# maxdoblas/QuickEd

Hardware: AMD Instinct MI355X
Metric: alignments/sec + GCUPS, 10kb x 10kb 5%-error pairs (higher is better)
Workload: dtype u64; 1 GPU; banded_score, DEVICE-RESIDENT inputs: 100000 pairs/GPU x 10000 bp @ 0.05 error, bandwidth 15 %, seeded generator (SURVEY 8d), ASCII already in HBM when the clock starts, results left in HBM (end-to-end rates: e2e); pairs_per_gpu=100000, length=10000, bandwidth=15, parallelism=pairs sharded over 1 GPU(s), no data-path collective

## Files before the change

### quicked_amd/csrc/qe_kernels.hip

```cpp
#include <type_traits>
#include <hip/hip_runtime.h>
#include "qe_types.h"
#include "qe_bounded.h"
#include "qe_search.h"
#include "qe_tags.h"
#include "qe_check.h"

namespace qe {

#define QE_ONES (~(u64)0)
#define QE_WAVE_IN_BLOCK() ((int)(threadIdx.x >> 6))
#define QE_GROUP_INDEX() ((int)(blockIdx.x * (blockDim.x >> 6) + (threadIdx.x >> 6)))
extern __shared__ uint4 qe_dyn_lds[];

__device__ __forceinline__ u32 lo32(u64 x) { return (u32)x; }
__device__ __forceinline__ u32 hi32(u64 x) { return (u32)(x >> 32); }
__device__ __forceinline__ u64 mk64(u32 lo, u32 hi) { return ((u64)hi << 32) | lo; }

__device__ __forceinline__ int64_t tile_elem(int col, int slot, int nslots) {
    return ((int64_t)(col >> 3) * nslots + slot) * 512 + (col & 7);
}

__device__ __forceinline__ int wave_min(int v) {
#pragma unroll
// ... 250 lines not shown
                u32 inP, inM;
                if (k == 0) { inP = __builtin_amdgcn_ubfe(hp, c, 1); inM = __builtin_amdgcn_ubfe(hm, c, 1); }
                else {
                    inP = (gP[k - 1] & 1u) | top[k];
                    inM = (gM[k - 1] & 1u) & ~top[k];
                }
                u32 phhi, mhhi;
                block_step_core(elo, ehi, Plo[k], Phi[k], Mlo[k], Mhi[k], inP, inM, phhi, mhhi);
                gP[k] = __builtin_amdgcn_alignbit(gP[k], phhi, 31);
                gM[k] = __builtin_amdgcn_alignbit(gM[k], mhhi, 31);
                if (k + 1 == K) asm("" : "+v"(Plo[k]) : "v"(gP[k]), "v"(gM[k]));
                if ((c & 15) == 15) {
                    if (act[k]) {
                        uint4* q = st + (int64_t)(2 * half + (c >> 4) + 1) * st_stride + k * 64;
                        if (c == 31 && half == 1) q = (k == 0) ? stl_first : stl + k * 64;
                        *q = make_uint4(Plo[k], Phi[k], Mlo[k], Mhi[k]);
                    }
                }
            }
        }
#pragma unroll
        for (int k = 0; k < K; ++k) {
            const u32 rP = __builtin_bitreverse32(gP[k]), rM = __builtin_bitreverse32(gM[k]);
            if (half) { oPhi[k] = rP; oMhi[k] = rM; } else { oPlo[k] = rP; oMlo[k] = rM; }
        }
    }
#pragma unroll
    for (int k = 0; k < K; ++k) {
        P[k] = mk64(Plo[k], Phi[k]); M[k] = mk64(Mlo[k], Mhi[k]);
        oP[k] = mk64(oPlo[k], oPhi[k]); oM[k] = mk64(oMlo[k], oMhi[k]);
    }
}

template <int K>
__device__ __forceinline__ void slots_pass(int nl, int i, int r, u64* Pv, u64* Mv, const int32_t* Srd, int32_t* Swr, int64_t stride,
                                           const u64* pp, int p0, u64 T0, u64 T1, u64& hinP, u64& hinM, u32& adv) {
    u64 P[K], M[K], a[K], b[K];
    int sc[K], v0[K];
#pragma unroll
    for (int k = 0; k < K; ++k) {
        P[k] = 0; M[k] = 0; a[k] = 0; b[k] = 0; sc[k] = 0;
        if (k < nl) {
            u64 nn;
            P[k] = Pv[(int64_t)(i + k) * stride]; M[k] = Mv[(int64_t)(i + k) * stride]; sc[k] = Srd[(int64_t)(r + k) * stride];
            load_planes(pp, p0 + 64 * (r + k), a[k], b[k], nn);
        }
        v0[k] = __popcll(P[k]) - __popcll(M[k]);
    }
    u64 houtP, houtM;
    run64_skew<K>(P, M, a, b, T0, T1, hinP, hinM, houtP, houtM);
    if (nl > 0) {
        int d = __popcll(houtP) - __popcll(houtM);
#pragma unroll
        for (int k = K - 1; k >= 0; --k) {
            if (k < nl) {
                Swr[(int64_t)(r + k) * stride] = sc[k] + d;
                Pv[(int64_t)(i + k - 1) * stride] = P[k]; Mv[(int64_t)(i + k - 1) * stride] = M[k];
            }
            d -= (__popcll(P[k]) - __popcll(M[k])) - v0[k];
        }
        adv += 64u * (u32)nl;
    }
    hinP = houtP; hinM = houtM;
}

__device__ __forceinline__ void run64_win2(u64& P0, u64& M0, u64& P1, u64& M1, u64 a0, u64 b0, u64 a1, u64 b1, u64 T0, u64 T1,
                                           u64 hinP, bool patch, u64 Eq_x, u64& gP, u64& gM, uint4* st, int st_stride) {
    const u32 a0lo = lo32(a0), a0hi = hi32(a0), b0lo = lo32(b0), b0hi = hi32(b0);
    const u32 a1lo = lo32(a1), a1hi = hi32(a1), b1lo = lo32(b1), b1hi = hi32(b1);
    u32 P0lo = lo32(P0), P0hi = hi32(P0), M0lo = lo32(M0), M0hi = hi32(M0);
    u32 P1lo = lo32(P1), P1hi = hi32(P1), M1lo = lo32(M1), M1hi = hi32(M1);
    u32 oPlo = 0, oPhi = 0, oMlo = 0, oMhi = 0;
#pragma unroll 1
    for (int half = 0; half < 2; ++half) {
        const u32 t0 = half ? hi32(T0) : lo32(T0), t1 = half ? hi32(T1) : lo32(T1);
        const u32 hp = half ? hi32(hinP) : lo32(hinP);
        u32 g0P = 0, g0M = 0;
        u32 m0[32], m1[32];
#pragma unroll
        for (int s = 0; s < 33; ++s) {
            if (s < 32) {
                m0[s] = (u32)__builtin_amdgcn_sbfe((int)t0, s, 1);
                m1[s] = (u32)__builtin_amdgcn_sbfe((int)t1, s, 1);
            }
            if (s >= 1) {
                const int c = s - 1;
                if ((c & 7) == 0) st[(4 * half + (c >> 3)) * st_stride] = make_uint4(P1lo, P1hi, M1lo, M1hi);
                u32 inP = g0P & 1u, inM = g0M & 1u;
                if (c == 31 && half == 1 && patch) {
// ... 343 lines not shown
    Geom g;
    const int kend = abs(n - m) + 1;
    g.cutoff = max(max(kend, cutoff_in), 65);
    g.diff = m - n;
    const int rel = (g.cutoff - abs(g.diff) + 1) / 2;
    if (g.diff >= 0) {
        g.prolog = (rel + 63) / 64;
        g.ebb = (rel + g.diff + 63) / 64 + 1 + g.prolog;
    } else {
        g.prolog = (rel - g.diff + 63) / 64;
        g.ebb = (rel + 63) / 64 + 1 + g.prolog;
    }
    g.fin = g.prolog * 64 + g.diff;
    return g;
}

struct GroupWs {
    u64* Pv; u64* Mv; int32_t* S; int16_t* cf; int16_t* cl;
};
__device__ __forceinline__ GroupWs group_ws(uint8_t* ws, int64_t off, int ns, int nrows, int nch) {
    GroupWs w;
    uint8_t* p = ws + off;
    w.Pv = (u64*)p;              p += (int64_t)(ns + 1) * 64 * 8;
    w.Mv = (u64*)p;              p += (int64_t)(ns + 1) * 64 * 8;
    w.S = (int32_t*)p;           p += (int64_t)nrows * 64 * 4;
    w.cf = (int16_t*)p;          p += (int64_t)nch * 64 * 2;
    w.cl = (int16_t*)p;
    return w;
}

#ifndef QE_FILL_K
#define QE_FILL_K 3
#endif
template <bool FILL>
__global__ __launch_bounds__(512) void k_banded(BandedArgs A) {
    const int g = QE_GROUP_INDEX(), lane = threadIdx.x & 63, t = g * 64 + lane;
    if (g * 64 >= A.T.ntasks) return;
    int pair = (t < A.T.ntasks) ? A.T.pair[t] : -1;
    if (A.only_if != nullptr && pair >= 0 && A.only_if[t] == 0) pair = -1;
    const bool valid = pair >= 0;
    if (!__any(valid)) return;
    int m = 1, n = 1, p0 = 0, t0 = 0, cut_in = 0, tfin = 0, prune = 0x7fffffff;
    const u64* pp = A.P.pl_p;
    const u64* tp = A.P.pl_t;
    u32 fl = 0;
    if (valid) {
        m = A.T.m[t]; n = A.T.n[t]; p0 = A.T.p0[t]; t0 = A.T.t0[t];
        cut_in = A.T.cutoff[t];
        tfin = FILL ? n : A.T.tfin[t];
        if (!FILL && A.prune != nullptr) prune = A.prune[t];
        pp = A.P.pl_p + A.P.pl_p_off[pair];
        tp = A.P.pl_t + A.P.pl_t_off[pair];
        fl = A.P.flags[pair];
    }
    const bool hasN = (fl & FLAG_HAS_N) != 0;
    const Geom G = band_geometry(m, n, cut_in);
    const int thr = prune < cut_in ? prune : G.cutoff;
    const int nw = (m + 63) >> 6;
    const bool fgeom = FILL || A.fill_geom != 0;
    const int nsl = fgeom ? G.ebb : ((G.cutoff + 63) >> 6) + 1;
    const int stop_row = fgeom ? nw - 1 : nw;
    const int lvl_last = (m - 1) & 63;
    int first = G.prolog, last = nsl - 1, pos_v = -G.prolog, pos_h = 0;
    int max_row_init = nsl - 1;
    u32 adv = 0;

    const int gns = A.g_nslots[g], gnr = A.g_nrows[g], gnch = A.g_nch[g];
    const GroupWs W = group_ws(A.ws, A.g_ws_off[g], gns, gnr, gnch);
    u64* const Pv = W.Pv + 64 + lane;
    u64* const Mv = W.Mv + 64 + lane;
    int32_t* const S = W.S + lane;
    uint4* const cp = FILL ? A.mat + A.g_mat_off[g] + lane : nullptr;
    const int64_t cps = (int64_t)gns * 64;
    uint4* const hw = FILL ? cp + (int64_t)QE_CPC * gnch * cps : nullptr;

    for (int s = 0; s < gns; ++s) {
        if (valid && s < nsl) {
            Pv[(int64_t)s * 64] = QE_ONES;
            Mv[(int64_t)s * 64] = 0;
            S[(int64_t)s * 64] = 64 * (s + 1);
            if (FILL) cp[(int64_t)s * 64] = make_uint4(~0u, ~0u, 0u, 0u);
        }
    }
    if (FILL && valid) { W.cf[lane] = (int16_t)first; W.cl[lane] = (int16_t)last; }

    const int nfull = tfin >> 6, tail = tfin & 63;
    const int my_chunks = valid ? nfull + (tail ? 1 : 0) : 0;
    const int wave_chunks = wave_max(my_chunks);

    for (int k = 0; k < wave_chunks; ++k) {
        const int ncols = (k < nfull) ? 64 : ((k == nfull) ? tail : 0);
        const bool on = valid && ncols > 0;
        u64 T0 = 0, T1 = 0, TN = 0;
        if (on) load_planes(tp, t0 + 64 * k, T0, T1, TN);
        const int rhi = min(last, nw - 1 - pos_v);
        const int fmin = wave_min(on ? first : 0x7fffffff), fmax = wave_max(on ? first : -0x7fffffff);
        const bool rel = A.lane_rel != 0 && fmin < fmax;
        const int ib = rel ? (on ? first : 0) : 0;
        const int i0 = rel ? 0 : fmin;
        const int i1 = rel ? wave_max(on ? rhi - first : -0x7fffffff) : wave_max(on ? rhi : -0x7fffffff);
        u64 hinP = QE_ONES, hinM = 0;
        u64 qP = 0, qM = 0, qa0 = 0, qb0 = 0, qa1 = 0, qb1 = 0;
        int qS = 0, qi = -0x7fffffff;
        const int psh = p0 & 63;
        const bool unaligned = __any(psh != 0);
        auto prefetch = [&](int j) {
            const int jc = min(max(j, 0), gns - 1), rc = min(max(j + pos_v, 0), gnr - 1), rp = min(max(j + pos_v, 0), nw);
            qP = Pv[(int64_t)jc * 64]; qM = Mv[(int64_t)jc * 64]; qS = S[(int64_t)rc * 64];
            const u64* w = pp + 3 * (int64_t)((p0 >> 6) + rp);
            qa0 = w[0]; qb0 = w[1];
            if (unaligned) { qa1 = w[3]; qb1 = w[4]; }
            qi = j;
        };
        if (FILL) prefetch(i0 + ib);
        for (int x = i0; x <= i1; ++x) {
            const int i = x + ib;
            const bool act = on && i >= first && i <= rhi;
            const int r = i + pos_v;
            if (!FILL) {
                const int lo = on ? first : 0x7fffffff, hi_ = on ? rhi : -0x7fffffff;
                const bool plain = !(on && (ncols != 64 || hasN));
                int nl = 0;
                auto planned = [&](int K) {
                    bool bad;
                    nl = pass_plan(i, K, lo, hi_, r, nw, plain, A.score_masked != 0, bad);
                    return !__any(bad);
                };
                if (i == first) { hinP = QE_ONES; hinM = 0; }
                if (x + 3 <= i1 && planned(4)) { slots_pass<4>(nl, i, r, Pv, Mv, S, S, 64, pp, p0, T0, T1, hinP, hinM, adv); x += 3; continue; }
                if (x + 1 <= i1 && planned(2)) { slots_pass<2>(nl, i, r, Pv, Mv, S, S, 64, pp, p0, T0, T1, hinP, hinM, adv); x += 1; continue; }
            }
            if (FILL && QE_FILL_K > 1 && A.fill_multi && x + QE_FILL_K - 1 <= i1) {
                constexpr int K = QE_FILL_K;
                bool actk[K], slowk = false;
                u32 topk[K];
#pragma unroll
                for (int q = 0; q < K; ++q) {
                    actk[q] = on && (i + q) >= first && (i + q) <= rhi;
                    topk[q] = ((i + q) == first) ? 1u : 0u;
                    slowk |= actk[q] && (ncols != 64 || hasN || (i + q + pos_v) == nw - 1);
                }
                if (!__any(slowk)) {
                    u64 P[K], M[K], a[K], b[K], oP[K], oM[K];
                    int sc[K];
#pragma unroll
                    for (int q = 0; q < K; ++q) {
                        P[q] = 0; M[q] = 0; a[q] = 0; b[q] = 0; sc[q] = 0;
                        if (actk[q]) {
                            u64 nn;
                            P[q] = Pv[(int64_t)(i + q) * 64]; M[q] = Mv[(int64_t)(i + q) * 64]; sc[q] = S[(int64_t)(r + q) * 64];
                            load_planes(pp, p0 + 64 * (r + q), a[q], b[q], nn);
                        }
                    }
                    if (i == first) { hinP = QE_ONES; hinM = 0; }
                    uint4* const st0 = cp + (int64_t)(QE_CPC * k) * cps + (int64_t)i * 64;
                    uint4* const stl0 = cp + (int64_t)(QE_CPC * k + QE_CPC) * cps + (int64_t)(i - 1) * 64;
                    run64_skew_fill<K>(P, M, a, b, T0, T1, hinP, hinM, oP, oM, actk, topk, st0, cps,
                                       (i == 0) ? st0 + QE_CPC * cps : stl0, stl0);
#pragma unroll
                    for (int q = 0; q < K; ++q) {
                        if (actk[q]) {
                            const u64 iP = (q == 0) ? hinP : (topk[q] ? QE_ONES : oP[q > 0 ? q - 1 : 0]);
                            const u64 iM = (q == 0) ? hinM : (topk[q] ? (u64)0 : oM[q > 0 ? q - 1 : 0]);
                            hw[((int64_t)k * gns + (i + q)) * 64] = make_uint4(lo32(iP), hi32(iP), lo32(iM), hi32(iM));
                            S[(int64_t)(r + q) * 64] = sc[q] + __popcll(oP[q]) - __popcll(oM[q]);
                            Pv[(int64_t)(i + q - 1) * 64] = P[q]; Mv[(int64_t)(i + q - 1) * 64] = M[q];
                            adv += 64u;
                        }
                    }
                    hinP = oP[K - 1]; hinM = oM[K - 1];
                    x += K - 1;
                    continue;
                }
            }
            u64 P = 0, M = 0, a = 0, b = 0, nn = 0;
            int sc = 0;
            if (FILL) {
                if (qi != i) prefetch(i);
                if (act) {
                    P = qP; M = qM; sc = qS;
                    a = (qa0 >> psh) | ((qa1 << 1) << (63 - psh));
                    b = (qb0 >> psh) | ((qb1 << 1) << (63 - psh));
                    if (hasN || r == nw - 1) load_planes(pp, p0 + 64 * r, a, b, nn);
                }
                prefetch(i + 1);
            } else if (act) {
                P = Pv[(int64_t)i * 64];
                M = Mv[(int64_t)i * 64];
                sc = S[(int64_t)r * 64];
                load_planes(pp, p0 + 64 * r, a, b, nn);
            }
            if (i == first) { hinP = QE_ONES; hinM = 0; }
            const bool lastblk = (r == nw - 1);
            uint4* st = nullptr; uint4* st_last = nullptr;
            if (FILL) {
                st = cp + (int64_t)(QE_CPC * k) * cps + (int64_t)i * 64;
                st_last = cp + (int64_t)(QE_CPC * k + QE_CPC) * cps + (int64_t)(i - 1) * 64;
                if (i == 0) st_last = st + QE_CPC * cps;
                if (act) hw[((int64_t)k * gns + i) * 64] = make_uint4(lo32(hinP), hi32(hinP), lo32(hinM), hi32(hinM));
            }
            u64 houtP, houtM, sP, sM;
            const bool slow = act && (ncols != 64 || hasN || lastblk);
            if (!__any(slow)) {
                run64_fast<FILL ? 2 : 0, true>(P, M, a, b, T0, T1, hinP, hinM, houtP, houtM, act, st, cps, st_last);
                sP = houtP; sM = houtM;
            } else {
                run64_general<FILL ? 2 : 0>(P, M, a, b, nn, T0, T1, TN, hinP, hinM, houtP, houtM, sP, sM,
                                            lastblk ? lvl_last : 63, act ? ncols : 0, true, st, cps, st_last);
            }
            if (act) {
                sc += __popcll(sP) - __popcll(sM);
                S[(int64_t)r * 64] = sc;
                const int64_t dst = (ncols == 64) ? (int64_t)(i - 1) * 64 : (int64_t)i * 64;
                Pv[dst] = P;
                Mv[dst] = M;
                adv += (u32)ncols;
            }
            hinP = houtP; hinM = houtM;
        }
        if (on && ncols == 64) {
            const bool c1 = (first + 2 < last) && (G.fin > 64 * (first + 1));
            bool cut_lo = false;
            if (c1) cut_lo = S[(int64_t)(first + pos_v + 1) * 64] + (G.fin - 64 * (first + 1)) > thr;
            if (cut_lo && pos_h >= G.prolog) first++;
            else if (!cut_lo && pos_h < G.prolog) first--;
            Pv[(int64_t)last * 64] = QE_ONES;
            Mv[(int64_t)last * 64] = 0;
            if (FILL) cp[(int64_t)(QE_CPC * k + QE_CPC) * cps + (int64_t)last * 64] = make_uint4(~0u, ~0u, 0u, 0u);
            const int pos = last + pos_v;
            S[(int64_t)(pos + 1) * 64] = S[(int64_t)pos * 64] + 64;
            max_row_init = max(max_row_init, pos + 1);
            const bool c2 = (first + 2 < last) && (64 * (last - 1) > G.fin);
            bool cut_hi = false;
            if (c2) cut_hi = S[(int64_t)(last + pos_v - 1) * 64] + (64 * (last - 1) - G.fin) > thr;
            if (cut_hi || (pos_v + last >= stop_row)) last--;
            pos_v++;
            pos_h++;
            if (FILL) { W.cf[(int64_t)pos_h * 64 + lane] = (int16_t)first; W.cl[(int64_t)pos_h * 64 + lane] = (int16_t)last; }
        }
    }
    if (valid) {
        const int row = nw - 1;
        int score = -1;
        if (row <= max_row_init) {
            score = S[(int64_t)row * 64];
            if (m & 63) score -= 64 - (m & 63);
        }
        A.o_score[t] = score;
        A.o_first[t] = first;
        A.o_last[t] = last;
        A.o_posv[t] = pos_v;
        A.o_maxrow[t] = max_row_init;
        A.o_adv[t] = adv;
    }
}

template __global__ void k_banded<false>(BandedArgs);
template __global__ void k_banded<true>(BandedArgs);

#define QE_HAVE_K_BOUNDED_DIAG 1
__global__ __launch_bounds__(256) void k_bounded_diag(BoundedArgs A) {
    const int g = QE_GROUP_INDEX(), lane = threadIdx.x & 63, t = g * 64 + lane;
    if (g * 64 >= A.T.ntasks) return;
    const int pair = (t < A.T.ntasks) ? A.T.pair[t] : -1;
    const bool valid = pair >= 0;
    if (!__any(valid)) return;
    int m = 1, n = 1, bound = 0;
    const u64* pp = A.P.pl_p;
    const u64* tp = A.P.pl_t;
    BoundedDiag S;
    S.Pv = S.Mv = S.wa = S.wb = S.wn = S.xa = S.xb = S.xn = S.force = S.track = 0; S.score = 0; S.dlo = 0;
    if (valid) {
        m = A.T.m[t]; n = A.T.n[t]; bound = A.T.cutoff[t];
        pp = A.P.pl_p + A.P.pl_p_off[pair];
        tp = A.P.pl_t + A.P.pl_t_off[pair];
        bounded_diag_init(S, pp, m, n, bound);
    }
    const int my_chunks = valid ? (n + 63) >> 6 : 0;
    const int wave_chunks = wave_max(my_chunks);
    u32 adv = 0;
    for (int k = 0; k < wave_chunks; ++k) {
        const int ncols = (k < my_chunks) ? min(64, n - 64 * k) : 0;
        const bool live = ncols > 0 && S.score <= bound;
        if (!__any(live)) break;
        if (live) {
            const u64* q = tp + 3 * (int64_t)k;
            const u64 T0 = q[0], T1 = q[1], TN = q[2];
            bounded_diag_chunk(S, pp, m, k, ncols, T0, T1, TN);
            adv += (u32)ncols;
        }
    }
// ... 3311 lines not shown
```

### quicked_amd/csrc/qe_pool.h

```cpp
#pragma once
#include <hip/hip_runtime.h>

#include <sys/syscall.h>
#include <unistd.h>

#include <algorithm>
#include <atomic>
#include <chrono>
#include <cstdio>
#include <cstdlib>
#include <cstring>
#include <memory>
#include <mutex>
#include <shared_mutex>
#include <thread>
#include <vector>

namespace qe {

struct HipError { hipError_t e; const char* what; int line; };
#define HIP_CHECK(expr)                                                             \
    do {                                                                            \
        hipError_t e__ = (expr);                                                    \
        if (e__ != hipSuccess) throw qe::HipError{e__, #expr, __LINE__};            \
    } while (0)

struct Chip {
    int cus = 256, simds = 1024;
    size_t slots2() const { return (size_t)simds * 2; }
    size_t frac2(double f) const { return (size_t)((double)simds * 2.0 * f); }
};
inline const Chip& chip(int device) {
    static Chip table[16];
    static std::once_flag once[16];
    const int d = (device >= 0 && device < 16) ? device : 0;
    std::call_once(once[d], [d] {
        int cus = 0;
        if (hipDeviceGetAttribute(&cus, hipDeviceAttributeMultiprocessorCount, d) == hipSuccess && cus > 0) { table[d].cus = cus; table[d].simds = cus * 4; }
        else (void)hipGetLastError();
    });
    return table[d];
}

enum class Sw : int {
    QuickedFast, QuickedEst, QuickedScorePass, FinishMerge, FinishMergePairs, Finishers, LaneRel, CoopG, CoopFillG, CoopLds,
    CoopTallFill, Wave, ScoreSys, Stage3Device, FormatWave, WindowedCp, WindowedQuad, WindowedSys, SplitBytes, FillSys, FillMulti,
    TraceSys, Trace, TracePool, OomWaitMs, BoundedDiag, ScoreNarrow, NarrowFit, NarrowPrune, ScoreMasked, TagsWave, SearchForm, SearchHitsWsKb, Count
};
struct SwitchDef { Sw sw; const char* name; long long dflt; };
inline constexpr SwitchDef switch_defs[] = {
    {Sw::QuickedFast, "QE_QUICKED_FAST", 1},           {Sw::QuickedEst, "QE_QUICKED_EST", 0},
    {Sw::QuickedScorePass, "QE_QUICKED_SCORE_PASS", -1},
    {Sw::FinishMerge, "QE_FINISH_MERGE", 4},           {Sw::FinishMergePairs, "QE_FINISH_MERGE_PAIRS", 8192},
    {Sw::Finishers, "QE_FINISHERS", 3},                {Sw::LaneRel, "QE_LANE_REL", 1},
    {Sw::CoopG, "QE_COOP_G", 1},                       {Sw::CoopFillG, "QE_COOP_FILL_G", 1},
    {Sw::CoopLds, "QE_COOP_LDS", 1},                   {Sw::CoopTallFill, "QE_COOP_TALL_FILL", 1},
    {Sw::Wave, "QE_WAVE", -1},                         {Sw::ScoreSys, "QE_SCORE_SYS", -1},
    {Sw::Stage3Device, "QE_STAGE3_DEVICE", -1},        {Sw::FormatWave, "QE_FORMAT_WAVE", -1},
    {Sw::WindowedCp, "QE_WINDOWED_CP", 1},             {Sw::WindowedQuad, "QE_WINDOWED_QUAD", -1},
    {Sw::WindowedSys, "QE_WINDOWED_SYS", -1},          {Sw::SplitBytes, "QE_SPLIT_BYTES", 1LL << 24},
    {Sw::FillSys, "QE_FILL_SYS", -1},                  {Sw::FillMulti, "QE_FILL_MULTI", 1},
    {Sw::TraceSys, "QE_TRACE_SYS", -1},                {Sw::Trace, "QE_TRACE", 0},
    {Sw::TracePool, "QE_TRACE_POOL", 0},               {Sw::OomWaitMs, "QE_OOM_WAIT_MS", 10000},
    {Sw::BoundedDiag, "QE_BOUNDED_DIAG", -1},
    {Sw::ScoreNarrow, "QE_SCORE_NARROW", -1},
    {Sw::NarrowFit, "QE_NARROW_FIT", -1},
    {Sw::NarrowPrune, "QE_NARROW_PRUNE", -1},
    {Sw::ScoreMasked, "QE_SCORE_MASKED", 1},
    {Sw::TagsWave, "QE_TAGS_WAVE", -1},
    {Sw::SearchForm, "QE_SEARCH_FORM", -1},
    {Sw::SearchHitsWsKb, "QE_SEARCH_HITS_WS_KB", 262144},
};
inline constexpr int switch_count = (int)Sw::Count;
constexpr bool switch_rows_in_order() {
    for (int i = 0; i < switch_count; ++i) if ((int)switch_defs[i].sw != i) return false;
    return true;
}
static_assert(sizeof(switch_defs) / sizeof(switch_defs[0]) == (size_t)switch_count && switch_rows_in_order(), "one row per switch, in the order of Sw");

struct SwitchTable {
    bool set[switch_count];
    long long value[switch_count];
    SwitchTable() {
        for (int i = 0; i < switch_count; ++i) {
            const char* e = getenv(switch_defs[i].name);
            set[i] = e != nullptr;
            value[i] = e ? strtoll(e, nullptr, 10) : switch_defs[i].dflt;
        }
    }
};
inline std::atomic<const SwitchTable*> g_switches{nullptr};
inline const SwitchTable& switches() {
    const SwitchTable* t = g_switches.load(std::memory_order_acquire);
    if (!t) {
        const SwitchTable* fresh = new SwitchTable();
        if (g_switches.compare_exchange_strong(t, fresh, std::memory_order_acq_rel)) t = fresh;
        else delete fresh;
    }
    return *t;
}
inline void switches_reload() { g_switches.store(new SwitchTable(), std::memory_order_release); }
// ... 519 lines not shown
```

### quicked_amd/csrc/qe_stages.hip

```cpp
#pragma once

namespace qe {

template <class Args> static Args with_prio(Args a) { a.prio = 1; return a; }

template <typename Kernel, typename Args>
static void launch_groups(Context& C, Kernel kernel, const Args& args, size_t ngroups, int max_waves, size_t lds_per_wave, bool chain = false,
                          size_t pin_override = 0) {
    if (ngroups == 0) return;
    const int wpb = std::min(4, max_waves);
    const unsigned blocks = (unsigned)((ngroups + wpb - 1) / wpb);
    const Chip& chp = chip(C.device);
    size_t pin = ((size_t)blocks * (size_t)std::max(1, C.in_flight) > (size_t)chp.cus) ? (size_t)54 * 1024 : (size_t)84 * 1024;
    if (chain && (size_t)blocks * (size_t)std::max(1, C.in_flight) <= (size_t)chp.cus / 2) pin = (size_t)108 * 1024;
    if (pin_override) pin = pin_override;
    const size_t lds = std::max(pin, lds_per_wave * (size_t)wpb);
    static thread_local std::vector<std::pair<const void*, int>> configured;
    const void* fn = reinterpret_cast<const void*>(kernel);
    if (std::find(configured.begin(), configured.end(), std::make_pair(fn, tl_device)) == configured.end()) {
        HIP_CHECK(hipFuncSetAttribute(fn, hipFuncAttributeMaxDynamicSharedMemorySize, 160 * 1024));
        configured.emplace_back(fn, tl_device);
    }
    hipLaunchKernelGGL(kernel, dim3(blocks), dim3(64 * wpb), lds, C.stream, args);
    HIP_CHECK(hipGetLastError());
// ... 181 lines not shown
    return b;
}

static BandedArgs score_args(const quicked_batch& B, const ScoreLaunch& S, bool reversed) {
    BandedArgs a{};
    a.score_masked = sw(Sw::ScoreMasked);
    a.P = pair_view(B, reversed); a.T = S.T.v;
    a.ws = S.D.ws; a.g_ws_off = S.D.ws_off; a.g_nslots = S.D.nslots; a.g_nrows = S.D.nrows; a.g_nch = S.D.nch;
    a.g_mat_off = S.D.mat_off;
    a.o_score = S.O.score; a.o_first = S.O.first; a.o_last = S.O.last; a.o_posv = S.O.posv; a.o_adv = S.O.adv; a.o_maxrow = S.O.len;
    return a;
}

static ScoreLaunch launch_banded_score(quicked_batch& B, Context& C, const TaskList& L, bool reversed, int timed, bool fill_geom = false,
                                       const int32_t* d_cut = nullptr, const int32_t* d_skip = nullptr) {
    ScoreLaunch S;
    S.nt = L.pair.size();
    BandLayout lay = band_layout(L, fill_geom, false);
    lay.mat_u4 = 0;
    S.T = upload_tasks(L, C);
    S.D = upload_layout(lay, C);
    S.O = take_out(C, S.nt);
    if (d_cut) apply_device_cutoffs(C, S.T, S.nt, S.O.score, d_cut, d_skip);
    BandedArgs a = score_args(B, S, reversed);
    a.lane_rel = sw(Sw::LaneRel);
    a.fill_geom = fill_geom ? 1 : 0;
    auto* ke = timed ? C.kernel_events(timed - 1) : nullptr;
    if (ke) HIP_CHECK(hipEventRecord(ke->first, C.stream));
    launch_groups(C, k_banded<false>, a, L.ngroups(), 8, 0);
    if (ke) HIP_CHECK(hipEventRecord(ke->second, C.stream));
    return S;
}

struct NarrowPlan { bool ok = false; int cls = 0; size_t live = 0, narrower = 0; };
static NarrowPlan narrow_plan(const TaskList& L) {
    NarrowPlan P;
    int n_max = 1;
    for (size_t t = 0; t < L.pair.size(); ++t) {
        if (L.pair[t] < 0) continue;
        if (L.tfin[t] != L.n[t]) return P;
        ++P.live;
        P.narrower += narrow_cutoff(L.m[t], L.n[t], L.cutoff[t]) != L.cutoff[t];
        n_max = std::max(n_max, L.n[t]);
    }
    while ((n_max >> (P.cls + 1)) != 0 && P.cls < 31) ++P.cls;
    P.ok = P.narrower > 0;
    return P;
}
enum : int { QE_NARROW_PROBE = 16 };
static int narrow_take(Context& C, int cls) {
    const int v = C.narrow_off[cls].load();
    if (v == 0) return 1;
    if (v >= QE_NARROW_PROBE) { C.narrow_off[cls] = 1; return sw(Sw::ScoreNarrow) == -2 ? 0 : 2; }
    C.narrow_off[cls] = v + 1;
    return 0;
}
enum : int { QE_NARROW_FIT_RUNS = 16 };
static int narrow_fit_q(Context& C, int cls, bool policy) {
    const int f = sw(Sw::NarrowFit);
    if (f >= 0) return f;
    if (!policy) return 0;
    int q = 0;
    for (auto& v : C.narrow_q[cls]) q = std::max(q, v.load());
    return q;
}
static int narrow_prune_q(Context& C, int cls, bool policy) {
    const int f = sw(Sw::NarrowPrune);
    if (f >= 0) return f;
    if (!policy || sw(Sw::NarrowFit) >= 0) return 0;
    int q = 0, lo = 0, reports = 0;
    for (auto& a : C.narrow_q[cls]) {
        const int v = a.load();
        if (v <= 0) continue;
        ++reports;
        q = std::max(q, v);
// ... 83 lines not shown
    S.T = upload_tasks(L, C);
    S.D = upload_layout(lay, C);
    S.O = take_out(C, S.nt);
    ScoreLaunch P;
    P.nt = Ls.pair.size();
    P.T = upload_tasks(Ls, C);
    P.D = upload_layout(lays, C);
    P.O = take_out(C, P.nt);
    S.narrow = C.scratch_p->take<unsigned long long>(QE_NARROW_STAT);
    S.narrow_probe = true;
    HIP_CHECK(hipMemsetAsync(S.narrow, 0, QE_NARROW_STAT * sizeof(unsigned long long), C.stream));
    hipStream_t main_s = C.stream, side = C.side_stream();
    HIP_CHECK(hipEventRecord(C.ev_fork, main_s)); HIP_CHECK(hipStreamWaitEvent(side, C.ev_fork, 0));
    BandedArgs a = score_args(B, S, reversed);
    a.lane_rel = sw(Sw::LaneRel);
    auto* ke = timed ? C.kernel_events(timed - 1) : nullptr;
    if (ke) HIP_CHECK(hipEventRecord(ke->first, main_s));
    launch_groups(C, k_banded<false>, a, L.ngroups(), 8, 0);
    if (ke) HIP_CHECK(hipEventRecord(ke->second, main_s));
    C.stream = side;
    BandedArgs b = score_args(B, P, reversed);
    b.lane_rel = a.lane_rel;
    launch_groups(C, k_banded<false>, b, Ls.ngroups(), 8, 0);
    C.stream = main_s;
    HIP_CHECK(hipEventRecord(C.ev_join, side)); HIP_CHECK(hipStreamWaitEvent(main_s, C.ev_join, 0));
    NarrowArgs x{};
    x.phase = 3; x.stride = QE_NARROW_PROBE;
    x.T = P.T.v; x.score = S.O.score; x.adv = S.O.adv; x.q_score = P.O.score; x.q_adv = P.O.adv; x.main_cutoff = S.T.cutoff; x.stat = S.narrow;
    hipLaunchKernelGGL(k_narrow, dim3((unsigned)((P.nt + 255) / 256)), dim3(256), 0, main_s, x);
    HIP_CHECK(hipGetLastError());
    return S;
}

static ScoreLaunch launch_banded_narrow(quicked_batch& B, Context& C, const TaskList& L, bool reversed, int timed, const BandLayout& lay, int q, int qp) {
    ScoreLaunch S;
    S.nt = L.pair.size();
    const size_t nt = S.nt;
    S.T = upload_tasks(L, C);
    S.D = upload_layout(lay, C);
    S.O = take_out(C, nt);
    ScoreLaunch S2 = S;
    S2.O = take_out(C, nt);
    int32_t* blk = C.scratch_p->take<int32_t>(10 * nt);
    S.narrow = C.scratch_p->take<unsigned long long>(QE_NARROW_STAT);
    NarrowArgs x{};
    x.T = S.T.v; x.cut1 = blk; x.score = S.O.score; x.adv = S.O.adv;
    x.q_pair = blk + nt; x.q_p0 = blk + 2 * nt; x.q_m = blk + 3 * nt; x.q_t0 = blk + 4 * nt; x.q_n = blk + 5 * nt;
    x.q_cutoff = blk + 6 * nt; x.q_tfin = blk + 7 * nt; x.q_src = blk + 8 * nt;
    x.q_score = S2.O.score; x.q_adv = S2.O.adv; x.stat = S.narrow; x.q = q;
    x.qp = q > 0 ? qp : 0; x.prune1 = blk + 9 * nt;
    S2.T.v.pair = x.q_pair; S2.T.v.p0 = x.q_p0; S2.T.v.m = x.q_m; S2.T.v.t0 = x.q_t0; S2.T.v.n = x.q_n;
    S2.T.v.cutoff = x.q_cutoff; S2.T.v.tfin = x.q_tfin;
    const dim3 grid((unsigned)((nt + 255) / 256)), block(256);
    auto* ke = timed ? C.kernel_events(timed - 1) : nullptr;
    if (ke) HIP_CHECK(hipEventRecord(ke->first, C.stream));
    x.phase = 0;
    hipLaunchKernelGGL(k_narrow, grid, block, 0, C.stream, x);
    BandedArgs a = score_args(B, S, reversed);
    a.T.cutoff = x.cut1;
    if (x.qp > 0) a.prune = x.prune1;
    a.lane_rel = sw(Sw::LaneRel);
    launch_groups(C, k_banded<false>, a, L.ngroups(), 8, 0);
    x.phase = 1;
    hipLaunchKernelGGL(k_narrow, grid, block, 0, C.stream, x);
    BandedArgs b = score_args(B, S2, reversed);
    b.lane_rel = a.lane_rel;
    launch_groups(C, k_banded<false>, b, L.ngroups(), 8, 0);
    x.phase = 2;
    hipLaunchKernelGGL(k_narrow, grid, block, 0, C.stream, x);
    HIP_CHECK(hipGetLastError());
    if (ke) HIP_CHECK(hipEventRecord(ke->second, C.stream));
    return S;
}

static int coop_lanes(const TaskList& L, int in_flight = 1, bool fill = false) {
    const Sw force = fill ? Sw::CoopFillG : Sw::CoopG;
    const bool e = sw_set(force);
    int min_nsl = 1 << 30, n_max = 1;
    size_t live = 0;
    for (size_t t = 0; t < L.pair.size(); ++t) {
        if (L.pair[t] < 0) continue;
        ++live;
        const HGeom hg = host_geometry(L.m[t], L.n[t], L.cutoff[t]);
        min_nsl = std::min(min_nsl, fill ? hg.ebb : hg.ebb_local);
        n_max = std::max(n_max, L.n[t]);
    }
    if (live == 0) return 1;
    int G = 1;
    const Chip& chp = chip(tl_device);
    const size_t target = std::min<size_t>(2 * chp.slots2(), chp.frac2(0.34) * (size_t)std::max(1, n_max / 10000));
    if (e) G = sw(force);
    else
        while (G < 64 && ((live * G) / 64) * (size_t)std::max(1, in_flight) < target) G *= 2;
    while (G > 1 && min_nsl < 3 * G + 4) G /= 2;
// ... 210 lines not shown
    BandedArgs a = score_args(B, S, false);
    a.o_abort = S.O.hew; a.doubling = 1; a.o_cutoff = d_cut;
    launch_groups(C, k_banded_sys<6, false>, with_prio(a), nt, 4, 0, false, (size_t)40 * 1024);
    d2h(score, S.O.score, nt, C.stream); d2h(adv, S.O.adv, nt, C.stream); d2h(flagged, S.O.hew, nt, C.stream); d2h(cutoff, d_cut, nt, C.stream);
    HIP_CHECK(hipStreamSynchronize(C.stream));
    return true;
}

static void run_banded_score(quicked_batch& B, Context& C, const TaskList& L, bool reversed, StageResult* R,
                             bool fetch, int32_t** d_score_out, PendingFetch* pf = nullptr, bool narrow_ok = false) {
    const bool forced = sw_set(Sw::CoopG) || sw(Sw::Wave) == 1;
    const int lg = forced ? 0 : sys_score_lanes(L, fetch ? 1 : C.in_flight);
    const int G0 = lg ? 1 : coop_lanes(L, fetch ? 1 : C.in_flight);
    const bool wave = !lg && wave_form_wanted(L) && (G0 < 2 || sw(Sw::Wave) == 1);
    const int G = wave ? 1 : G0;
    const int nmode = narrow_ok ? sw(Sw::ScoreNarrow) : 0;
    NarrowPlan np;
    BandLayout ulay;
    bool narrow = false, policy = false, probe = false;
    auto fits = [&]() {
        const BandLayout own = band_layout(L, false, false);
        ulay = narrow_uniform(own);
        return ulay.ws_bytes <= 2 * own.ws_bytes;
    };
    if (nmode == 1) { np = narrow_plan(L); narrow = np.ok && fits(); }
    else if (nmode != 0 && !forced && !lg && !wave && G < 2 && (size_t)L.ngroups() >= (size_t)chip(C.device).simds) {
        np = narrow_plan(L);
        policy = np.ok && 2 * np.narrower >= np.live;
        const int take = policy ? narrow_take(C, np.cls) : 0;
        if (take == 1 && !fits()) policy = false;
        narrow = policy && take == 1;
        probe = policy && take == 2;
    }
    const ScoreLaunch S = narrow ? launch_banded_narrow(B, C, L, reversed, 1, ulay, narrow_fit_q(C, np.cls, policy), narrow_prune_q(C, np.cls, policy)) :
                          probe ? launch_banded_probe(B, C, L, reversed, 1) :
                          lg ? launch_banded_sys(B, C, L, reversed, lg, 1) :
                          wave ? launch_banded_wave(B, C, L, reversed, 1)
                               : ((G >= 2) ? launch_banded_coop(B, C, L, reversed, G, 1) : launch_banded_score(B, C, L, reversed, 1));
    if (d_score_out) *d_score_out = S.O.score;
    if (pf && !fetch) {
        pf->kind = 1; pf->task_pair = L.pair; pf->d_score = S.O.score; pf->d_adv = S.O.adv; pf->counter_slot = 0;
        pf->d_abort = (!narrow && !probe && G >= 2) ? S.O.hew : nullptr;
        pf->d_narrow = S.narrow; pf->narrow_ctx = policy ? &C : nullptr; pf->narrow_cls = np.cls; pf->narrow_probe = probe;
    }
    if (fetch && R) {
        FetchBatch fb(C);
        if (!narrow && !probe && G >= 2) fb.add(R->hew, S.O.hew, S.nt);
        fb.add(R->score, S.O.score, S.nt); fb.add(R->adv, S.O.adv, S.nt);
        if (S.narrow) fb.add(R->narrow, (const unsigned long long*)S.narrow, QE_NARROW_STAT);
        fb.sync();
        R->narrow_probe = probe;
        if (S.narrow && policy) narrow_report(&C, np.cls, R->narrow, probe);
    }
}

static bool quicked_score_pass_wanted() { return sw(Sw::QuickedScorePass) != 0; }
static bool quicked_score_pass_fits(const TaskList& L, bool fetch) {
    if (sw(Sw::QuickedScorePass) == 1 || !fetch) return true;
    if (sys_score_lanes(L, 1, true) != 0) return true;
    size_t live = 0;
    for (int32_t pr : L.pair) live += pr >= 0;
    return live >= (size_t)chip(tl_device).simds * 4;
}
static void run_fill_score(quicked_batch& B, Context& C, const TaskList& L, StageResult* R, bool fetch, int32_t** d_score_out,
                           PendingFetch* pf = nullptr, const int32_t* d_cut = nullptr, const int32_t* d_skip = nullptr) {
    const int lg = sys_score_lanes(L, fetch ? 1 : C.in_flight, true);
    const ScoreLaunch S = lg ? launch_banded_sys(B, C, L, false, lg, 2 , true, d_cut, d_skip)
// ... 1002 lines not shown
```

### quicked_amd/csrc/qe_types.h

```cpp
#pragma once
#include <stdint.h>

namespace qe {

typedef uint64_t u64;
typedef uint32_t u32;

enum : u32 { FLAG_HAS_N = 1u, FLAG_NONCANON = 2u };
enum : int { QE_CP_COLS = 16, QE_CPC = 64 / QE_CP_COLS };
enum : u32 { OP_M = 0, OP_X = 1, OP_I = 2, OP_D = 3 };

struct PairView {
    const uint8_t* asc_p;  const int64_t* asc_p_off;  const int32_t* p_len;
    const uint8_t* asc_t;  const int64_t* asc_t_off;  const int32_t* t_len;
    const u64* pl_p;  const int64_t* pl_p_off;
    const u64* pl_t;  const int64_t* pl_t_off;
    const u32* flags;
};

struct TaskView {
    int32_t ntasks;
    const int32_t* pair;
    const int32_t* p0;  const int32_t* m;
    const int32_t* t0;  const int32_t* n;
// ... 6 lines not shown
    const uint8_t* asc;  const int64_t* asc_off;  const int32_t* len;
    u64* planes;  const int64_t* pl_off;
    u32* flags;
    int32_t reverse;
};

struct WireArgs {
    int32_t nseq, wire;
    const u64* words;  const int64_t* w_off;  const int32_t* len;
    u64* planes;  const int64_t* pl_off;
    u32* flags;
};
struct RevArgs {
    int32_t nseq;
    const u64* fwd;  u64* rev;  const int64_t* pl_off;  const int32_t* len;
};

struct BandedArgs {
    PairView P;
    TaskView T;
    uint8_t* ws;  const int64_t* g_ws_off;  const int32_t* g_nslots;  const int32_t* g_nrows;  const int32_t* g_nch;
    uint4* mat;  const int64_t* g_mat_off;
    int32_t* o_score;  int32_t* o_first;  int32_t* o_last;  int32_t* o_posv;  u32* o_adv;  int32_t* o_maxrow;
    const int32_t* only_if;
    int32_t fill_multi = 1;
    int32_t lane_rel = 1;
    int32_t score_masked = 1;
    int32_t* o_abort = nullptr;
    int32_t doubling = 0;
    int32_t* o_cutoff = nullptr;
    int32_t prio = 0;
    int32_t fill_geom = 0;
    const int32_t* prune = nullptr;
};

struct BoundedArgs {
    PairView P;
    TaskView T;
    int32_t* o_score;
    u32* o_adv;
};

struct SearchArgs {
    PairView P;
    TaskView T;
    int32_t mode, flags;
    const int32_t* in_score;  const int32_t* in_end;
    uint8_t* ws;  const int64_t* g_ws_off;  const int32_t* g_nb;
    int32_t* o_score;  int32_t* o_end;  int32_t* o_start;  u32* o_adv;
};

struct SearchHitsArgs {
    SearchArgs S;
    int32_t max_hits;
    int32_t* raw;
    int32_t* o_found;  int32_t* o_best;  int32_t* o_len;
};
struct HitExpandArgs {
    TaskView T;
    int32_t max_hits, infix;
    const int32_t* raw;
    const int32_t* len;  const int64_t* off;
    int32_t* hits;
    int32_t* o_pair;  int32_t* o_m;  int32_t* o_n;  int32_t* o_score;  int32_t* o_end;
};

// ... 118 lines not shown
}
QE_T_HD int narrow_fit_lane(int m, int n, int cutoff_in, int q, int s_g) {
    const int half = narrow_cutoff(m, n, cutoff_in);
    if (s_g <= 0 || s_g >= narrow_slots(m, n, half)) return half;
    const int c = narrow_fit_cutoff(m, n, cutoff_in, s_g);
    return (c > 0 && narrow_accepts(m, n, c, cutoff_in, narrow_rhat(q, cutoff_in))) ? c : half;
}
QE_T_HD int narrow_prune(int m, int n, int cutoff_in, int c1, int qp) {
    if (qp <= 0 || c1 == cutoff_in || c1 == narrow_cutoff(m, n, cutoff_in)) return c1;
    if (narrow_slots(m, n, c1) <= 3) return c1;
    const int r = narrow_rhat(qp, cutoff_in);
    return r < c1 ? r : c1;
}
QE_T_HD bool narrow_accepts_pruned(int m, int n, int c1, int cutoff_in, int p, int r) {
    return narrow_accepts(m, n, c1, cutoff_in, r) && r <= p;
}
QE_T_HD int narrow_ratio(int m, int n, int cutoff_in, int r) {
    if (!narrow_accepts(m, n, narrow_cutoff(m, n, cutoff_in), cutoff_in, r)) return -1;
    return (int)(((long long)r * 1024 + cutoff_in - 1) / cutoff_in);
}

QE_T_HD int pass_plan(int i, int K, int lo, int hi, int r, int nw, bool plain, bool masked, bool& fallback) {
    if (!masked) {
        const bool all = i >= lo && i + K - 1 <= hi, none = i + K - 1 < lo || i > hi;
        fallback = !(all || none) || (all && (!plain || r + K - 1 >= nw - 1));
        return all ? K : 0;
    }
    const int a0 = i > lo ? i : lo, a1 = i + K - 1 < hi ? i + K - 1 : hi;
    const int nl = a1 >= a0 ? a1 - a0 + 1 : 0;
    fallback = nl > 0 && (a0 != i || !plain || r + nl - 1 >= nw - 1);
    return nl;
}

enum : int { QE_NARROW_STAT = 6 };
struct NarrowArgs {
    int32_t phase, stride, q;
    TaskView T;
    int32_t* cut1;
    int32_t qp = 0;  int32_t* prune1 = nullptr;
    int32_t* score;  u32* adv;
    int32_t *q_pair, *q_p0, *q_m, *q_t0, *q_n, *q_cutoff, *q_tfin, *q_src;
    const int32_t* q_score;  const u32* q_adv;
    const int32_t* main_cutoff;
    unsigned long long* stat;
};

struct BandState {
    int32_t G;
    const uint8_t* ws;  const int64_t* g_ws_off;  const int32_t* g_nslots;  const int32_t* g_nrows;  const int32_t* g_nch;
    const int32_t* first;  const int32_t* last;  const int32_t* posv;  const int32_t* maxrow;
    const int32_t* abort;
};

struct JoinArgs {
    int32_t nnodes;
    const int32_t* m;  const int32_t* n1;  const int32_t* n2;
    BandState F, R;
    BandState Ffb, Rfb;
    int32_t* o_best;  int32_t* o_score_l;  int32_t* o_score_r;  int32_t* o_ok;
};

struct SegFormatArgs {
    int32_t npairs;
    const int64_t* seg_off;
    const int32_t* seg_kind;  const int32_t* seg_a;  const int32_t* seg_b;
    const u32* runs;  const int64_t* g_runs_off;  const int32_t* nruns;
// ... 27 lines not shown
```

Before: 21.01 million alignments/s.

## Keep narrow first-pass band state in LDS with a ring-buffered score array

Adds an LDS variant of the banded score kernel for the first launch of the two-pass narrow scoring path. Each wave keeps its Pv/Mv slot vectors in shared memory, along with a 16-entry ring of row scores indexed modulo the ring size, so these no longer live in the global group workspace. The variant applies only when the narrow band fits (at most 13 slots) and there are enough groups to fill the SIMDs; otherwise it falls back. Lanes whose band exceeds the LDS capacity are marked invalid and report -1. LDS use per block may reduce occupancy.

```diff
diff --git a/quicked_amd/csrc/qe_kernels.hip b/quicked_amd/csrc/qe_kernels.hip
--- a/quicked_amd/csrc/qe_kernels.hip
+++ b/quicked_amd/csrc/qe_kernels.hip
@@ -306,7 +306,7 @@
     }
 }
 
-template <int K>
+template <int K, bool RING = false>
 __device__ __forceinline__ void slots_pass(int nl, int i, int r, u64* Pv, u64* Mv, const int32_t* Srd, int32_t* Swr, int64_t stride,
                                            const u64* pp, int p0, u64 T0, u64 T1, u64& hinP, u64& hinM, u32& adv) {
     u64 P[K], M[K], a[K], b[K];
@@ -316,7 +316,7 @@
         P[k] = 0; M[k] = 0; a[k] = 0; b[k] = 0; sc[k] = 0;
         if (k < nl) {
             u64 nn;
-            P[k] = Pv[(int64_t)(i + k) * stride]; M[k] = Mv[(int64_t)(i + k) * stride]; sc[k] = Srd[(int64_t)(r + k) * stride];
+            P[k] = Pv[(int64_t)(i + k) * stride]; M[k] = Mv[(int64_t)(i + k) * stride]; sc[k] = Srd[(int64_t)(RING ? score_lds_row(r + k) : r + k) * stride];
             load_planes(pp, p0 + 64 * (r + k), a[k], b[k], nn);
         }
         v0[k] = __popcll(P[k]) - __popcll(M[k]);
@@ -328,7 +328,7 @@
 #pragma unroll
         for (int k = K - 1; k >= 0; --k) {
             if (k < nl) {
-                Swr[(int64_t)(r + k) * stride] = sc[k] + d;
+                Swr[(int64_t)(RING ? score_lds_row(r + k) : r + k) * stride] = sc[k] + d;
                 Pv[(int64_t)(i + k - 1) * stride] = P[k]; Mv[(int64_t)(i + k - 1) * stride] = M[k];
             }
             d -= (__popcll(P[k]) - __popcll(M[k])) - v0[k];
@@ -738,19 +738,21 @@
 #ifndef QE_FILL_K
 #define QE_FILL_K 3
 #endif
-template <bool FILL>
+#define QE_HAVE_K_BANDED_LDS 1
+template <bool FILL, bool LDS = false>
 __global__ __launch_bounds__(512) void k_banded(BandedArgs A) {
+    static_assert(!(FILL && LDS), "the fill's state stays in the group workspace");
     const int g = QE_GROUP_INDEX(), lane = threadIdx.x & 63, t = g * 64 + lane;
     if (g * 64 >= A.T.ntasks) return;
     int pair = (t < A.T.ntasks) ? A.T.pair[t] : -1;
     if (A.only_if != nullptr && pair >= 0 && A.only_if[t] == 0) pair = -1;
-    const bool valid = pair >= 0;
-    if (!__any(valid)) return;
+    const bool have = pair >= 0;
+    if (!__any(have)) return;
     int m = 1, n = 1, p0 = 0, t0 = 0, cut_in = 0, tfin = 0, prune = 0x7fffffff;
     const u64* pp = A.P.pl_p;
     const u64* tp = A.P.pl_t;
     u32 fl = 0;
-    if (valid) {
+    if (have) {
         m = A.T.m[t]; n = A.T.n[t]; p0 = A.T.p0[t]; t0 = A.T.t0[t];
         cut_in = A.T.cutoff[t];
         tfin = FILL ? n : A.T.tfin[t];
@@ -763,7 +765,7 @@
     const Geom G = band_geometry(m, n, cut_in);
     const int thr = prune < cut_in ? prune : G.cutoff;
     const int nw = (m + 63) >> 6;
-    const bool fgeom = FILL || A.fill_geom != 0;
+    const bool fgeom = FILL || (!LDS && A.fill_geom != 0);
     const int nsl = fgeom ? G.ebb : ((G.cutoff + 63) >> 6) + 1;
     const int stop_row = fgeom ? nw - 1 : nw;
     const int lvl_last = (m - 1) & 63;
@@ -771,11 +773,18 @@
     int max_row_init = nsl - 1;
     u32 adv = 0;
 
-    const int gns = A.g_nslots[g], gnr = A.g_nrows[g], gnch = A.g_nch[g];
-    const GroupWs W = group_ws(A.ws, A.g_ws_off[g], gns, gnr, gnch);
+    const int gns = LDS ? A.lds_slots : A.g_nslots[g], gnr = LDS ? 0 : A.g_nrows[g], gnch = LDS ? 0 : A.g_nch[g];
+    GroupWs W;
+    if (LDS) {
+        uint8_t* lb = (uint8_t*)qe_dyn_lds + (size_t)QE_WAVE_IN_BLOCK() * (size_t)score_lds_bytes(gns);
+        W.Pv = (u64*)lb; W.Mv = W.Pv + (gns + 1) * 64; W.S = (int32_t*)(W.Mv + (gns + 1) * 64); W.cf = nullptr; W.cl = nullptr;
+        if (nsl > gns) pair = -1;
+    } else W = group_ws(A.ws, A.g_ws_off[g], gns, gnr, gnch);
+    const bool valid = pair >= 0;
     u64* const Pv = W.Pv + 64 + lane;
     u64* const Mv = W.Mv + 64 + lane;
     int32_t* const S = W.S + lane;
+    auto srow = [](int r) { return (int64_t)(LDS ? score_lds_row(r) : r) * 64; };
     uint4* const cp = FILL ? A.mat + A.g_mat_off[g] + lane : nullptr;
     const int64_t cps = (int64_t)gns * 64;
     uint4* const hw = FILL ? cp + (int64_t)QE_CPC * gnch * cps : nullptr;
@@ -784,7 +793,7 @@
         if (valid && s < nsl) {
             Pv[(int64_t)s * 64] = QE_ONES;
             Mv[(int64_t)s * 64] = 0;
-            S[(int64_t)s * 64] = 64 * (s + 1);
+            S[srow(s)] = 64 * (s + 1);
             if (FILL) cp[(int64_t)s * 64] = make_uint4(~0u, ~0u, 0u, 0u);
         }
     }
@@ -812,7 +821,7 @@
         const bool unaligned = __any(psh != 0);
         auto prefetch = [&](int j) {
             const int jc = min(max(j, 0), gns - 1), rc = min(max(j + pos_v, 0), gnr - 1), rp = min(max(j + pos_v, 0), nw);
-            qP = Pv[(int64_t)jc * 64]; qM = Mv[(int64_t)jc * 64]; qS = S[(int64_t)rc * 64];
+            qP = Pv[(int64_t)jc * 64]; qM = Mv[(int64_t)jc * 64]; qS = S[srow(rc)];
             const u64* w = pp + 3 * (int64_t)((p0 >> 6) + rp);
             qa0 = w[0]; qb0 = w[1];
             if (unaligned) { qa1 = w[3]; qb1 = w[4]; }
@@ -833,8 +842,8 @@
                     return !__any(bad);
                 };
                 if (i == first) { hinP = QE_ONES; hinM = 0; }
-                if (x + 3 <= i1 && planned(4)) { slots_pass<4>(nl, i, r, Pv, Mv, S, S, 64, pp, p0, T0, T1, hinP, hinM, adv); x += 3; continue; }
-                if (x + 1 <= i1 && planned(2)) { slots_pass<2>(nl, i, r, Pv, Mv, S, S, 64, pp, p0, T0, T1, hinP, hinM, adv); x += 1; continue; }
+                if (x + 3 <= i1 && planned(4)) { slots_pass<4, LDS>(nl, i, r, Pv, Mv, S, S, 64, pp, p0, T0, T1, hinP, hinM, adv); x += 3; continue; }
+                if (x + 1 <= i1 && planned(2)) { slots_pass<2, LDS>(nl, i, r, Pv, Mv, S, S, 64, pp, p0, T0, T1, hinP, hinM, adv); x += 1; continue; }
             }
             if (FILL && QE_FILL_K > 1 && A.fill_multi && x + QE_FILL_K - 1 <= i1) {
                 constexpr int K = QE_FILL_K;
@@ -854,7 +863,7 @@
                         P[q] = 0; M[q] = 0; a[q] = 0; b[q] = 0; sc[q] = 0;
                         if (actk[q]) {
                             u64 nn;
-                            P[q] = Pv[(int64_t)(i + q) * 64]; M[q] = Mv[(int64_t)(i + q) * 64]; sc[q] = S[(int64_t)(r + q) * 64];
+                            P[q] = Pv[(int64_t)(i + q) * 64]; M[q] = Mv[(int64_t)(i + q) * 64]; sc[q] = S[srow(r + q)];
                             load_planes(pp, p0 + 64 * (r + q), a[q], b[q], nn);
                         }
                     }
@@ -869,7 +878,7 @@
                             const u64 iP = (q == 0) ? hinP : (topk[q] ? QE_ONES : oP[q > 0 ? q - 1 : 0]);
                             const u64 iM = (q == 0) ? hinM : (topk[q] ? (u64)0 : oM[q > 0 ? q - 1 : 0]);
                             hw[((int64_t)k * gns + (i + q)) * 64] = make_uint4(lo32(iP), hi32(iP), lo32(iM), hi32(iM));
-                            S[(int64_t)(r + q) * 64] = sc[q] + __popcll(oP[q]) - __popcll(oM[q]);
+                            S[srow(r + q)] = sc[q] + __popcll(oP[q]) - __popcll(oM[q]);
                             Pv[(int64_t)(i + q - 1) * 64] = P[q]; Mv[(int64_t)(i + q - 1) * 64] = M[q];
                             adv += 64u;
                         }
@@ -893,7 +902,7 @@
             } else if (act) {
                 P = Pv[(int64_t)i * 64];
                 M = Mv[(int64_t)i * 64];
-                sc = S[(int64_t)r * 64];
+                sc = S[srow(r)];
                 load_planes(pp, p0 + 64 * r, a, b, nn);
             }
             if (i == first) { hinP = QE_ONES; hinM = 0; }
@@ -916,7 +925,7 @@
             }
             if (act) {
                 sc += __popcll(sP) - __popcll(sM);
-                S[(int64_t)r * 64] = sc;
+                S[srow(r)] = sc;
                 const int64_t dst = (ncols == 64) ? (int64_t)(i - 1) * 64 : (int64_t)i * 64;
                 Pv[dst] = P;
                 Mv[dst] = M;
@@ -927,29 +936,29 @@
         if (on && ncols == 64) {
             const bool c1 = (first + 2 < last) && (G.fin > 64 * (first + 1));
             bool cut_lo = false;
-            if (c1) cut_lo = S[(int64_t)(first + pos_v + 1) * 64] + (G.fin - 64 * (first + 1)) > thr;
+            if (c1) cut_lo = S[srow(first + pos_v + 1)] + (G.fin - 64 * (first + 1)) > thr;
             if (cut_lo && pos_h >= G.prolog) first++;
             else if (!cut_lo && pos_h < G.prolog) first--;
             Pv[(int64_t)last * 64] = QE_ONES;
             Mv[(int64_t)last * 64] = 0;
             if (FILL) cp[(int64_t)(QE_CPC * k + QE_CPC) * cps + (int64_t)last * 64] = make_uint4(~0u, ~0u, 0u, 0u);
             const int pos = last + pos_v;
-            S[(int64_t)(pos + 1) * 64] = S[(int64_t)pos * 64] + 64;
+            S[srow(pos + 1)] = S[srow(pos)] + 64;
             max_row_init = max(max_row_init, pos + 1);
             const bool c2 = (first + 2 < last) && (64 * (last - 1) > G.fin);
             bool cut_hi = false;
-            if (c2) cut_hi = S[(int64_t)(last + pos_v - 1) * 64] + (64 * (last - 1) - G.fin) > thr;
+            if (c2) cut_hi = S[srow(last + pos_v - 1)] + (64 * (last - 1) - G.fin) > thr;
             if (cut_hi || (pos_v + last >= stop_row)) last--;
             pos_v++;
             pos_h++;
             if (FILL) { W.cf[(int64_t)pos_h * 64 + lane] = (int16_t)first; W.cl[(int64_t)pos_h * 64 + lane] = (int16_t)last; }
         }
     }
-    if (valid) {
+    if (have) {
         const int row = nw - 1;
         int score = -1;
-        if (row <= max_row_init) {
-            score = S[(int64_t)row * 64];
+        if (valid && row <= max_row_init) {
+            score = S[srow(row)];
             if (m & 63) score -= 64 - (m & 63);
         }
         A.o_score[t] = score;
@@ -963,6 +972,7 @@
 
 template __global__ void k_banded<false>(BandedArgs);
 template __global__ void k_banded<true>(BandedArgs);
+template __global__ void k_banded<false, true>(BandedArgs);
 
 #define QE_HAVE_K_BOUNDED_DIAG 1
 __global__ __launch_bounds__(256) void k_bounded_diag(BoundedArgs A) {
diff --git a/quicked_amd/csrc/qe_pool.h b/quicked_amd/csrc/qe_pool.h
--- a/quicked_amd/csrc/qe_pool.h
+++ b/quicked_amd/csrc/qe_pool.h
@@ -45,7 +45,7 @@
 enum class Sw : int {
     QuickedFast, QuickedEst, QuickedScorePass, FinishMerge, FinishMergePairs, Finishers, LaneRel, CoopG, CoopFillG, CoopLds,
     CoopTallFill, Wave, ScoreSys, Stage3Device, FormatWave, WindowedCp, WindowedQuad, WindowedSys, SplitBytes, FillSys, FillMulti,
-    TraceSys, Trace, TracePool, OomWaitMs, BoundedDiag, ScoreNarrow, NarrowFit, NarrowPrune, ScoreMasked, TagsWave, SearchForm, SearchHitsWsKb, Count
+    TraceSys, Trace, TracePool, OomWaitMs, BoundedDiag, ScoreNarrow, NarrowFit, NarrowPrune, ScoreMasked, ScoreLds, TagsWave, SearchForm, SearchHitsWsKb, Count
 };
 struct SwitchDef { Sw sw; const char* name; long long dflt; };
 inline constexpr SwitchDef switch_defs[] = {
@@ -67,6 +67,7 @@
     {Sw::NarrowFit, "QE_NARROW_FIT", -1},
     {Sw::NarrowPrune, "QE_NARROW_PRUNE", -1},
     {Sw::ScoreMasked, "QE_SCORE_MASKED", 1},
+    {Sw::ScoreLds, "QE_SCORE_LDS", -1},
     {Sw::TagsWave, "QE_TAGS_WAVE", -1},
     {Sw::SearchForm, "QE_SEARCH_FORM", -1},
     {Sw::SearchHitsWsKb, "QE_SEARCH_HITS_WS_KB", 262144},
diff --git a/quicked_amd/csrc/qe_stages.hip b/quicked_amd/csrc/qe_stages.hip
--- a/quicked_amd/csrc/qe_stages.hip
+++ b/quicked_amd/csrc/qe_stages.hip
@@ -237,7 +237,7 @@
     return S;
 }
 
-struct NarrowPlan { bool ok = false; int cls = 0; size_t live = 0, narrower = 0; };
+struct NarrowPlan { bool ok = false; int cls = 0; size_t live = 0, narrower = 0; int slots1 = 0; };
 static NarrowPlan narrow_plan(const TaskList& L) {
     NarrowPlan P;
     int n_max = 1;
@@ -245,7 +245,9 @@
         if (L.pair[t] < 0) continue;
         if (L.tfin[t] != L.n[t]) return P;
         ++P.live;
-        P.narrower += narrow_cutoff(L.m[t], L.n[t], L.cutoff[t]) != L.cutoff[t];
+        const int c1 = narrow_cutoff(L.m[t], L.n[t], L.cutoff[t]);
+        P.narrower += c1 != L.cutoff[t];
+        P.slots1 = std::max(P.slots1, narrow_slots(L.m[t], L.n[t], c1));
         n_max = std::max(n_max, L.n[t]);
     }
     while ((n_max >> (P.cls + 1)) != 0 && P.cls < 31) ++P.cls;
@@ -395,7 +397,18 @@
     return S;
 }
 
-static ScoreLaunch launch_banded_narrow(quicked_batch& B, Context& C, const TaskList& L, bool reversed, int timed, const BandLayout& lay, int q, int qp) {
+static int score_lds_slots(const Context& C, const TaskList& L, int bound) {
+#ifndef QE_HAVE_K_BANDED_LDS
+    (void)C; (void)L; (void)bound;
+    return 0;
+#else
+    const int mode = sw(Sw::ScoreLds);
+    if (mode == 0 || (mode != 1 && (size_t)L.ngroups() < (size_t)chip(C.device).simds)) return 0;
+    return score_lds_fits(bound) ? bound : 0;
+#endif
+}
+
+static ScoreLaunch launch_banded_narrow(quicked_batch& B, Context& C, const TaskList& L, bool reversed, int timed, const BandLayout& lay, int q, int qp, int slots1) {
     ScoreLaunch S;
     S.nt = L.pair.size();
     const size_t nt = S.nt;
@@ -423,6 +436,12 @@
     a.T.cutoff = x.cut1;
     if (x.qp > 0) a.prune = x.prune1;
     a.lane_rel = sw(Sw::LaneRel);
+    a.lds_slots = score_lds_slots(C, L, slots1);
+    if (trace_on()) fprintf(stderr, "[qe] two-pass score: first launch of %d groups, band state in %s (%d slots)\n", L.ngroups(), a.lds_slots ? "LDS" : "the group workspace", a.lds_slots);
+#ifdef QE_HAVE_K_BANDED_LDS
+    if (a.lds_slots) launch_groups(C, k_banded<false, true>, a, L.ngroups(), 8, (size_t)score_lds_bytes(a.lds_slots));
+    else
+#endif
     launch_groups(C, k_banded<false>, a, L.ngroups(), 8, 0);
     x.phase = 1;
     hipLaunchKernelGGL(k_narrow, grid, block, 0, C.stream, x);
@@ -699,7 +718,7 @@
         narrow = policy && take == 1;
         probe = policy && take == 2;
     }
-    const ScoreLaunch S = narrow ? launch_banded_narrow(B, C, L, reversed, 1, ulay, narrow_fit_q(C, np.cls, policy), narrow_prune_q(C, np.cls, policy)) :
+    const ScoreLaunch S = narrow ? launch_banded_narrow(B, C, L, reversed, 1, ulay, narrow_fit_q(C, np.cls, policy), narrow_prune_q(C, np.cls, policy), np.slots1) :
                           probe ? launch_banded_probe(B, C, L, reversed, 1) :
                           lg ? launch_banded_sys(B, C, L, reversed, lg, 1) :
                           wave ? launch_banded_wave(B, C, L, reversed, 1)
diff --git a/quicked_amd/csrc/qe_types.h b/quicked_amd/csrc/qe_types.h
--- a/quicked_amd/csrc/qe_types.h
+++ b/quicked_amd/csrc/qe_types.h
@@ -62,6 +62,7 @@
     int32_t prio = 0;
     int32_t fill_geom = 0;
     const int32_t* prune = nullptr;
+    int32_t lds_slots = 0;
 };
 
 struct BoundedArgs {
@@ -246,6 +247,12 @@
     return nl;
 }
 
+QE_T_HD int score_lds_ring() { return 16; }
+QE_T_HD int score_lds_cap() { return score_lds_ring() - 3; }
+QE_T_HD bool score_lds_fits(int slots) { return slots >= 1 && slots <= score_lds_cap(); }
+QE_T_HD int score_lds_row(int r) { return r & (score_lds_ring() - 1); }
+QE_T_HD int score_lds_bytes(int slots) { return 2 * (slots + 1) * 64 * 8 + score_lds_ring() * 64 * 4; }
+
 enum : int { QE_NARROW_STAT = 6 };
 struct NarrowArgs {
     int32_t phase, stride, q;
```

Result: faster. 21.49 million alignments/s (median of 6 runs) (+2.3%).
